# uci-rendering/psdr-cuda

Measured on AMD Instinct MI355X. Metric: Mpath-samples/s renderC+renderD, cbox 512x512 spp=64; grad rel-L2 vs ref, higher is better.
Workload: dtype f32; 1 GPU; cbox 512x512 spp=64/GPU PathTracer(max_depth=3): renderC + configure + renderD + enoki.forward w.r.t. diffuse albedo, through the psdr_cuda surface; triangles=12, global_spp=64, world_size=1, device=AMD Radeon Graphics, local_rank=0

## Files before the change

### psdr-cuda_amd/csrc/psdr_collocated.hip

```cpp
#ifndef PSDR_WIDE_TREE
#if PSDR_VARIANT_FLAGS == 6
#define PSDR_WIDE_TREE 1
#else
#define PSDR_WIDE_TREE 0
#endif
#endif
#ifndef PSDR_LEAF_PAIR
#if PSDR_VARIANT_FLAGS == 6
#define PSDR_LEAF_PAIR 1
#else
#define PSDR_LEAF_PAIR 0
#endif
#endif
#include "psdr_kernels.h"
#include "psdr_collocated.h"

#ifndef PSDR_VARIANT_FLAGS
#error "compile with -DPSDR_VARIANT_FLAGS=0|1|2|3|4|6|8|10"
#endif
#define PSDR_CAT2(a, b) a##b
#define PSDR_CAT(a, b) PSDR_CAT2(a, b)

namespace {

// ... 134 lines not shown
    const long long nceil = (n + kBlock - 1) / kBlock * kBlock;
    for (long long j = (long long) blockIdx.x * kBlock + threadIdx.x; j < nceil; j += (long long) gridDim.x * kBlock) {
        float w[4] = {0.f, 0.f, 0.f, 0.f};
        int edge = -1;
        if (j < n) edge = collocated_edge_reverse_values<FL>(cx.sc, st, cx.jump, (uint64_t) (i0 + (order ? (long long) order[j] : j)), inv_sppe, adj_img, nrays, w);
        const bool head = wave_run_sum<4>(edge, w);
        if (head && edge >= 0) {
#pragma unroll
            for (int i = 0; i < 4; ++i) sink.add_pedge(edge, i, w[i]);
        }
    }
    count_rays(counters, nrays);
}

template <class G, class R, int FL>
int colloc_run_camera(psdr_scene_s *h, const psdr_render_opts *o, const TV<R, FL> &tv, float *img, float *dimg, hipStream_t s) {
    const long long WH = (long long) h->desc.width * h->desc.height;
    const int nsp = o->spp_end - o->spp_begin;
    if (o->spp <= 0 || nsp <= 0) return 0;
    LaunchCtx cx;
    if (int rc = make_ctx(h, o, 0, cx)) return rc;
    const long long n = WH * nsp;
    h->slots[0] += (uint64_t) n;
    const int own = (h->opt.own_pixels != 0 && nsp <= 64 && 64 % nsp == 0) ? 1 : 0;
    hipLaunchKernelGGL(HIP_KERNEL_NAME(k_colloc_camera<G, R, FL>), dim3(launch_blocks(h, n, camera_blocks_per_cu(h, n))), dim3(kBlock), lds_bytes(cx, h), s, cx, tv, o->spp, o->spp_begin,
                       SlotDiv(nsp), n, 1.f / (float) o->spp, img, dimg, WH * 3, h->d_counters, own);
    HIP_TRY(hipGetLastError());
    return 0;
}

template <int FL>
int colloc_render_c(psdr_scene_s *h, const psdr_render_opts *o, float *out_img, hipStream_t s) {
    const TangentView<0, FL> tv0{};
    return colloc_run_camera<float, float, FL>(h, o, tv0, out_img, nullptr, s);
}

template <int K, int FL>
int colloc_render_fwd_k(psdr_scene_s *h, const psdr_render_opts *o, const psdr_tangents *tangents, float *img, float *dimg, hipStream_t s) {
    const long long WH = (long long) h->desc.width * h->desc.height;
    TangentView<K, FL> tv;
    for (int k = 0; k < K; ++k) tv.t[k] = tangents[k];
    HIP_TRY(hipMemsetAsync(img, 0, sizeof(float) * WH * 3, s));
    HIP_TRY(hipMemsetAsync(dimg, 0, sizeof(float) * WH * 3 * K, s));
    bool geo = false;
    for (int k = 0; k < K; ++k) geo = geo || tangents[k].d_tri_info || tangents[k].d_cam_to_world;
    if (geo) { if (int rc = colloc_run_camera<Dual<K>, Dual<K>, FL>(h, o, tv, img, dimg, s)) return rc; }
    else { if (int rc = colloc_run_camera<float, Dual<K>, FL>(h, o, tv, img, dimg, s)) return rc; }
// ... 95 lines not shown
```

### psdr-cuda_amd/csrc/psdr_hip.hip

```cpp
#define PSDR_WIDE_TREE 2
#include "psdr_host.h"
#include "psdr_bvh_build.h"

#include <cstdlib>
#include <cstring>
#include <rocprim/rocprim.hpp>

namespace {
__global__ __launch_bounds__(kBlock) void k_trace(LaunchCtx cx, int m, const float *__restrict__ ox, const float *__restrict__ oy,
                                                  const float *__restrict__ oz, const float *__restrict__ dx,
                                                  const float *__restrict__ dy, const float *__restrict__ dz,
                                                  const float *__restrict__ tmax, int32_t *__restrict__ out_shape,
                                                  int32_t *__restrict__ out_tri, float *__restrict__ out_u, float *__restrict__ out_v) {
    TraversalStack st; setup_lds(cx, st);
    const SceneView &sc = cx.sc;
    for (int i = blockIdx.x * kBlock + threadIdx.x; i < m; i += gridDim.x * kBlock) {
        const Hit h = closest_hit<false, -1>(sc, st, Vec3f{ox[i], oy[i], oz[i]}, Vec3f{dx[i], dy[i], dz[i]}, tmax[i]);
        out_tri[i] = h.tri;
        out_shape[i] = h.tri >= 0 ? (sc.d.tri_mesh[h.tri] & ~PSDR_TRI_FACE_NORMALS) : -1;
        out_u[i] = h.u; out_v[i] = h.v;
    }
}


// ... 527 lines not shown
    }
    return L;
}

int ensure_tree_kind(psdr_scene_s *h, hipStream_t s) {
    if (!h->have_bvh || h->num_nodes <= 0) return 0;
    if (forest_tables(h) && !small_tables_fit(h)) return psdr_bvh_build(h, s);
    const bool forest = h->n_blas > 0;
    if (use_wide_tree(h, forest) == h->wide) return 0;
    std::vector<BvhNode> host_nodes((size_t) h->num_nodes);
    HIP_TRY(hipMemcpyAsync(host_nodes.data(), h->d_nodes, host_nodes.size() * sizeof(BvhNode), hipMemcpyDeviceToHost, s));
    HIP_TRY(hipStreamSynchronize(s));
    std::vector<int32_t> roots;
    if (forest) for (int k = 0; k < h->n_blas; ++k) { int32_t r; std::memcpy(&r, &h->blas_lo[k].w, 4); roots.push_back(r); }
    else roots.push_back(h->root);
    return bvh4_build(h, host_nodes, roots, forest, s);
}

int begin_call(psdr_scene_s *h, hipStream_t s) {
    h->last_stream = s;
    if (int rc = ensure_tree_kind(h, s)) return rc;
    h->slots[0] = h->slots[1] = h->slots[2] = 0; h->last_path_depth = 0;
    HIP_TRY(hipMemsetAsync(h->d_counters, 0, sizeof(unsigned long long) * kRayCounters * kRayCounterStride, s));
    return 0;
}


int primary_edge_order(psdr_scene_s *h, const LaunchCtx &cx, long long i0, long long n, const uint32_t **order, hipStream_t s) {
    *order = nullptr;
    if (!h->sort_edges || n < 65536 || n > 0x7fffffffLL) return 0;
    size_t temp = 0;
    const unsigned long long tiles = (unsigned long long) ((cx.sc.d.width + 7) >> 3) * (unsigned long long) ((cx.sc.d.height + 7) >> 3);
    unsigned tile_bits = 0;
    while ((1ull << tile_bits) < tiles) ++tile_bits;
    if (tile_bits + 6 >= 32) return 0;
    const unsigned end_bit = tile_bits + 7;
    const uint32_t invalid_key = 1u << (tile_bits + 6);
    uint32_t *nul = nullptr;
    HIP_TRY(rocprim::radix_sort_pairs(nullptr, temp, nul, nul, nul, nul, (size_t) n, 0, end_bit, s));
    const size_t need = 4 * sizeof(uint32_t) * (size_t) n + temp + 256;
    if (int rc = scratch_reserve(&h->d_sort, &h->sort_bytes, need, s, "primary-edge sort scratch")) return rc;
    uint32_t *k_in = reinterpret_cast<uint32_t *>(h->d_sort), *k_out = k_in + n, *v_in = k_out + n, *v_out = v_in + n;
    void *tmp = reinterpret_cast<void *>((reinterpret_cast<uintptr_t>(v_out + n) + 255) & ~(uintptr_t) 255);
    hipLaunchKernelGGL(k_primary_edge_keys, dim3((unsigned) ((n + kBlock - 1) / kBlock)), dim3(kBlock), 0, s, cx.sc, cx.jump, i0, n, k_in, v_in, invalid_key);
    HIP_TRY(hipGetLastError());
    HIP_TRY(rocprim::radix_sort_pairs(tmp, temp, k_in, k_out, v_in, v_out, (size_t) n, 0, end_bit, s));
// ... 303 lines not shown
    else if (n == "emitter_pretest") h->opt.emitter_pretest = iv;
    else if (n == "occ_rows") { h->opt.occ_rows = iv; h->have_bvh = false; }
    else if (n == "aa_prims") { h->aa_enabled = iv != 0; h->have_bvh = false; }
    else if (n == "tiny_scene") h->tiny_enabled = iv != 0;
    else if (n == "two_level") h->two_level_enabled = iv != 0;
    else if (n == "wf_binned") h->wf_binned = iv != 0;
    else if (n == "wf_traced") h->traced_enabled = iv != 0;
    else if (n == "bvh_build") h->bvh_device_mode = iv;
    else if (n == "sort_edges") h->sort_edges = iv != 0;
    else if (n == "blocks_per_cu") h->opt.blocks_per_cu = iv;
    else if (n == "camera_blocks") h->opt.camera_blocks = iv;
    else if (n == "tiny_variants") h->opt.tiny_variants = iv;
    else if (n == "wide") h->opt.wide = iv;
    else if (n == "lds_budget") h->opt.lds_budget = iv;
    else if (n == "sink_rep") h->opt.sink_rep = std::max(1, std::min(16, iv));
    else if (n == "sink_private") h->opt.sink_private = iv;
    else if (n == "rev_split") h->opt.rev_split = iv;
    else if (n == "tangent_live") h->opt.tangent_live = iv;
    else if (n == "wf_geo") h->opt.wf_geo = iv;
    else if (n == "logd") h->opt.logd = iv;
    else if (n == "seed_cache") h->opt.seed_cache = iv;
    else if (n == "logd_park") h->opt.logd_park = iv;
    else if (n == "seed_cache_log2") h->opt.seed_cache_log2 = std::max(0, std::min(40, iv));
    else if (n == "keep_records") h->opt.keep_records = iv;
    else if (n == "rev_sorted") h->opt.rev_sorted = iv;
    else if (n == "sedge_split") h->opt.sedge_split = iv;
    else if (n == "pt_sedge") h->opt.pt_sedge = iv & 3;
    else if (n == "pt_sedge_walk") h->opt.pt_sedge_walk = iv;
    else if (n == "probe") h->opt.probe = iv;
    else if (n == "trace_wg2") h->opt.trace_wg2 = iv;
    else if (n == "chunk_log2") h->opt.chunk_log2 = std::max(0, std::min(30, iv));
    else if (n == "bvh_maxleaf") h->opt.bvh_maxleaf = std::max(1, std::min(8, iv));
    else if (n == "bvh_tcost") h->opt.bvh_tcost = (float) value;
    else return fail("psdr_scene_set_option: unknown option '" + n + "'");
    h->kept.valid = false;
    if (n == "tiny_scene" || n == "two_level" || n == "bvh_build" || n == "wide" || n == "bvh_maxleaf" || n == "bvh_tcost" || n == "tiny_variants") h->have_bvh = false;
    return 0;
}

int psdr_scene_destroy(psdr_scene_t h) {
    if (!h) return 0;
    if (h->d_nodes) (void) hipFree(h->d_nodes);
    if (h->d_btris) (void) hipFree(h->d_btris);
    if (h->d_counters) (void) hipFree(h->d_counters);
    if (h->d_refit_area) (void) hipFree(h->d_refit_area);
    if (h->d_sort) (void) hipFree(h->d_sort);
// ... 299 lines not shown
int psdr_trace(psdr_scene_t h, int32_t m, const float *ox, const float *oy, const float *oz, const float *dx, const float *dy,
               const float *dz, const float *tmax, int32_t *out_shape, int32_t *out_tri, float *out_u, float *out_v, void *stream) {
    if (!h || !h->have_tables) return fail("Scene not loaded yet!");
    if (!h->have_bvh) return fail("Input scene must be configured!");
    if (m <= 0) return 0;
    LaunchCtx cx{};
    cx.sc.d = h->desc; cx.sc.nodes = h->d_nodes; cx.sc.btris = h->d_btris; cx.sc.root = h->root;
    fill_top(h, cx.sc);
    plan_lds(h, cx);
    hipLaunchKernelGGL(k_trace, dim3(launch_blocks(h, m)), dim3(kBlock), lds_bytes(cx, h), (hipStream_t) stream, cx, m, ox, oy, oz, dx, dy, dz, tmax,
                       out_shape, out_tri, out_u, out_v);
    HIP_TRY(hipGetLastError());
    return 0;
}

int psdr_render_c(psdr_scene_t h, const psdr_render_opts *o, float *out_img, void *stream) {
    if (!h || !o || !out_img) return fail("psdr_render_c: null argument");
    if (!h->have_tables) return fail("Scene not loaded yet!");
    if (int rc = check_counts(h, o)) return rc;
    if (int rc = check_microfacet(h, o)) return rc;
    hipStream_t s = (hipStream_t) stream;
    if (int rc = begin_call(h, s)) return rc;
    if (o->integrator == PSDR_INTEGRATOR_PATH) h->last_path_depth = o->max_depth;
    const long long WH = (long long) h->desc.width * h->desc.height;
    HIP_TRY(hipMemsetAsync(out_img, 0, sizeof(float) * WH * 3, s));
    if (o->integrator == PSDR_INTEGRATOR_COLLOCATED) return collocated_of(h)->render_c(h, o, out_img, s);
    return variant_of(h)->render_c(h, o, out_img, s);
}

int psdr_render_d_fwd(psdr_scene_t h, const psdr_render_opts *o, int32_t K, const psdr_tangents *tangents, float *out_img,
                      float *out_dimg, void *stream) {
    if (!h || !o || !out_img || !out_dimg || !tangents) return fail("psdr_render_d_fwd: null argument");
    if (!h->have_tables) return fail("Scene not loaded yet!");
    if (int rc = check_counts(h, o)) return rc;
    if (int rc = check_microfacet(h, o)) return rc;
    if (int rc = check_path_sedges(o)) return rc;
    hipStream_t s = (hipStream_t) stream;
    if (int rc = begin_call(h, s)) return rc;
    if (K != 1 && K != 3) return fail("psdr_render_d_fwd: K must be 1 or 3");
    if (o->integrator == PSDR_INTEGRATOR_COLLOCATED) return collocated_of(h)->render_fwd(h, o, K, tangents, out_img, out_dimg, s);
    if (int rc = variant_of(h)->render_fwd(h, o, K, tangents, out_img, out_dimg, s)) return rc;
    return path_sedge_of(h)->fwd(h, o, K, tangents, out_dimg, s);
}

int psdr_render_d_rev(psdr_scene_t h, const psdr_render_opts *o, const float *adj_img, float *out_img, const psdr_grads *grads,
                      void *stream) {
    if (!h || !o || !adj_img || !grads) return fail("psdr_render_d_rev: null argument");
    if (!h->have_tables) return fail("Scene not loaded yet!");
    if (int rc = check_counts(h, o)) return rc;
// ... 158 lines not shown
```

### psdr-cuda_amd/csrc/psdr_host.h

```cpp
#pragma once
#include "psdr_device.h"
#include "psdr_reverse.h"

#include <algorithm>
#include <type_traits>
#include <cmath>
#include <cstdio>
#include <cstdlib>
#include <cstring>
#include <string>
#include <vector>

using namespace psdr;

struct LaunchCtx {
    SceneView sc;
    LiParams lp;
    RngJump jump;
    int32_t off_stack;
    int32_t off_pathrec;
    int32_t off_sink;
    int32_t off_park;
};

// ... 93 lines not shown
    int tiny_variants = 1;
    int wide = -1;
    int lds_budget = 0;
    int sink_rep = 4;
    int sink_private = 1;
    int rev_split = -1;
    int tangent_live = 1;
    int wf_geo = 1;
    int own_pixels = 1;
    int emitter_pretest = 1;
    int occ_rows = 1;
    int logd = 1;
    int keep_records = 1;
    int rev_sorted = 1;
    int pt_sedge = 3;
    int pt_sedge_walk = 1;
    int sedge_split = -1;
    int chunk_log2 = 0;
    int probe = 1;
    int trace_wg2 = -1;
    int seed_cache = 1;
    int seed_cache_log2 = 25;
    int logd_park = 1;
    int bvh_maxleaf = 4;
    float bvh_tcost = 2.0f;
};

struct psdr_scene_s {
    psdr_scene_options opt;
    psdr_scene_desc desc{};
    bool have_tables = false;
    bool has_rough = true;
    int num_cus = 256;
    int lds_limit = 64 * 1024;

    BvhNode *d_nodes = nullptr;
    float4 *d_btris = nullptr;
    size_t cap_nodes = 0, cap_btris = 0;
    int32_t root = 0;
    bool have_bvh = false;
    int bvh_depth = 0, num_nodes = 0, num_btris = 0;
    Bvh4Node *d_nodes4 = nullptr;
    int32_t *d_topo4 = nullptr;
    size_t cap_nodes4 = 0;
    int num_nodes4 = 0, stack_need4 = 0;
    bool wide = false;
// ... 33 lines not shown
    std::vector<int32_t> emitter_i;
    int32_t *d_hot_map = nullptr, *d_hot_tris = nullptr;
    uint32_t *d_occ = nullptr; size_t occ_cap = 0; bool have_occ = false; int occ_max_rows = 0;
    int hot_rows = 0;
    bool hot_identity = false;
    size_t hot_cap = 0;

    bool sort_edges = true;
    void *d_sort = nullptr;
    size_t sort_bytes = 0;

    void *d_pe_rep = nullptr;
    size_t pe_rep_bytes = 0;

    void *d_rev_deep = nullptr;
    size_t rev_deep_bytes = 0;

    void *d_se_list = nullptr;
    size_t se_list_bytes = 0;

    void *d_rev = nullptr;
    size_t rev_bytes = 0;
    void *d_logd_bad = nullptr; size_t logd_bad_bytes = 0;
    struct KeptRecords { bool valid = false; psdr_render_opts o{}; uint64_t gen = 0; long long n = 0; int kind = 0; } kept;
    uint64_t tables_gen = 0;

    void *d_seed = nullptr;
    size_t seed_cap = 0;
    long long seed_key[4] = {0, 0, 0, 0};
    bool seed_valid = false;
    hipStream_t seed_stream = nullptr;
    hipEvent_t seed_event = nullptr;
    long long seed_fills = 0, seed_launches = 0;
    long long logd_launches = 0, logd_lean_launches = 0, logd_lean_seeded = 0;
    int logd_lean_lds = 0, logd_lean_park = 0;
    void *d_ws = nullptr;
    size_t ws_bytes = 0;
    void *d_live = nullptr;
    size_t live_bytes = 0;
    void *d_probe = nullptr;
    size_t probe_bytes = 0;
    uint32_t emit_rows = 0;
    int forest_min_inline = 0;
    int32_t pg_reso[3] = {1, 1, 1};
    const float *pg_cmf = nullptr, *pg_pmf = nullptr;
    float pg_sum = 0.f;
// ... 79 lines not shown
```

### psdr-cuda_amd/csrc/psdr_kernels.h

```cpp
#pragma once
#include "psdr_host.h"

namespace {
using namespace psdr_host;

__device__ __forceinline__ float wave_shfl_down(float v, int off) { return __shfl_down(v, off, 64); }

template <int CTRL, int ROW_MASK> __device__ __forceinline__ float dpp_add(float v) {
    return v + __int_as_float(__builtin_amdgcn_update_dpp(0, __float_as_int(v), CTRL, ROW_MASK, 0xf, true));
}
__device__ __forceinline__ float wave_total(float v) {
    v = dpp_add<0x111, 0xf>(v); v = dpp_add<0x112, 0xf>(v); v = dpp_add<0x114, 0xf>(v); v = dpp_add<0x118, 0xf>(v);
    v = dpp_add<0x142, 0xa>(v); v = dpp_add<0x143, 0xc>(v);
    return __int_as_float(__builtin_amdgcn_readlane(__float_as_int(v), 63));
}
#ifndef PSDR_DPP_ALWAYS
#define PSDR_DPP_ALWAYS 0
#endif
template <int N, bool DPP = (N <= 6 || PSDR_DPP_ALWAYS)> __device__ __forceinline__ bool wave_segmented_sum(int key, float (&v)[N]) {
    const int lane = threadIdx.x & 63;
    if (DPP && __ballot(key != __builtin_amdgcn_readfirstlane(key)) == 0ull) {
#pragma unroll
        for (int i = 0; i < N; ++i) v[i] = wave_total(v[i]);
        return lane == 0;
// ... 161 lines not shown
                                                   unsigned long long *counters, int own, const ulonglong2 *__restrict__ seed) {
    static_assert((FL & kScenePre) == 0, "seeded launches have no probe rows");
    constexpr long long j0 = 0;
    const ProbeView pv{nullptr, nullptr};
    PSDR_CAMERA_KERNEL_BODY(PSDR_SEED_LOAD, (((void) slot), camera_sample<G, R, INTEG>(cx.sc, tv, st, cx.lp, seeded_rng(sd, cx.jump), pixel, nrays)))
}
#undef PSDR_CAMERA_KERNEL_BODY
#undef PSDR_SEED_LOAD
#undef PSDR_SEED_LOAD_NONE

template <int K>
__global__ __launch_bounds__(kBlock) void k_logd_check(const float *__restrict__ texels, TangentView<K, 0> tv, int n, unsigned long long *counters, int *bad) {
    const int i = blockIdx.x * kBlock + threadIdx.x;
    bool b = false;
    if (i < n) {
        bool moved = false;
#pragma unroll
        for (int k = 0; k < K; ++k) moved = moved || tv.t[k].d_texels[i] != 0.f;
        b = moved && !(fabsf(texels[i]) > 1e-20f);
    }
    if (__ballot(b) != 0ull && (threadIdx.x & 63) == 0) atomicOr(bad, 1);
}
__global__ void k_logd_gate(unsigned long long *counters, const int *bad) { if (threadIdx.x == 0 && blockIdx.x == 0) counters[kLogdGateWord] = *bad ? 0ull : 1ull; }
template <int K, int FL, bool NOTREE>
__global__ __launch_bounds__(kBlock, ((PSDR_LOGD_WAVES_K1 > 0 && K == 1 && NOTREE) ? PSDR_LOGD_WAVES_K1 : camera_waves<float, Dual<K>, PSDR_INTEGRATOR_PATH, FL, NOTREE>())) void k_camera_logd(LaunchCtx cx, TV<Dual<K>, FL> tv, int spp, int s_begin, SlotDiv nsp,
                                                   long long n, float inv_spp, float *__restrict__ img, float *__restrict__ dimg, long long plane, unsigned long long *counters, int own) {
    constexpr int NV = 3 * (1 + K);
    if (counters[kLogdGateWord] != 1ull) return;
    TraversalStack st; setup_lds(cx, st, tv);
    uint32_t nrays = 0;
    const long long nceil = (n + kBlock - 1) / kBlock * kBlock;
    for (long long j = (long long) blockIdx.x * kBlock + threadIdx.x; j < nceil; j += (long long) gridDim.x * kBlock) {
        const bool in = j < n;
        int pixel = 0x7fffffff, s_in = 0;
        if (in) slot_to_pixel(j, nsp, pixel, s_in);
        float v[NV];
#pragma unroll
        for (int i = 0; i < NV; ++i) v[i] = 0.f;
        if (in) {
            const uint64_t slot = (uint64_t) pixel * (uint64_t) spp + (uint64_t) (s_begin + s_in);
            const Vec3<Dual<K>> r = camera_sample_logd<K>(cx.sc, tv, st, cx.lp, cx.jump, pixel, slot, nrays);
            v[0] = r.x.v * inv_spp; v[1] = r.y.v * inv_spp; v[2] = r.z.v * inv_spp;
#pragma unroll
            for (int k = 0; k < K; ++k) { v[3 + 3 * k] = r.x.d[k] * inv_spp; v[4 + 3 * k] = r.y.d[k] * inv_spp; v[5 + 3 * k] = r.z.d[k] * inv_spp; }
        }
        const bool head = wave_segmented_sum<NV>(pixel, v);
// ... 1277 lines not shown
}
inline const ulonglong2 *seed_table(psdr_scene_s *h, const psdr_render_opts *o, long long WH, int nsp, long long n, hipStream_t s) {
    if (h->opt.seed_cache == 0 || n <= 0 || n > (1ll << std::max(0, std::min(40, h->opt.seed_cache_log2)))) return nullptr;
    const long long key[4] = {WH, (long long) o->spp, (long long) o->spp_begin, (long long) nsp};
    if (h->d_seed != nullptr && h->seed_valid && std::equal(key, key + 4, h->seed_key)) {
        if (s != h->seed_stream && h->seed_event != nullptr && hipStreamWaitEvent(s, h->seed_event, 0) != hipSuccess) { (void) hipGetLastError(); return nullptr; }
        return reinterpret_cast<const ulonglong2 *>(h->d_seed);
    }
    h->seed_valid = false;
    if ((size_t) n > h->seed_cap) {
        if (h->d_seed) { (void) hipFreeAsync(h->d_seed, s); h->d_seed = nullptr; h->seed_cap = 0; }
        void *nb = nullptr;
        if (hipMallocAsync(&nb, (size_t) n * sizeof(ulonglong2), s) != hipSuccess) { (void) hipGetLastError(); return nullptr; }
        h->d_seed = nb; h->seed_cap = (size_t) n;
    }
    if (h->seed_event == nullptr && hipEventCreateWithFlags(&h->seed_event, hipEventDisableTiming) != hipSuccess) { (void) hipGetLastError(); h->seed_event = nullptr; return nullptr; }
    hipLaunchKernelGGL(k_seed_fill, dim3((unsigned) ((n + kBlock - 1) / kBlock)), dim3(kBlock), 0, s, reinterpret_cast<ulonglong2 *>(h->d_seed), n, o->spp, o->spp_begin, SlotDiv(nsp));
    if (hipGetLastError() != hipSuccess || hipEventRecord(h->seed_event, s) != hipSuccess) { (void) hipGetLastError(); return nullptr; }
    std::copy(key, key + 4, h->seed_key);
    h->seed_valid = true; h->seed_stream = s; h->seed_fills++;
    return reinterpret_cast<const ulonglong2 *>(h->d_seed);
}
template <class G, class R, int FL> constexpr bool seeded_render_c() { return (FL & kSceneTiny) != 0 && (FL & kScenePre) == 0 && std::is_same<G, float>::value && std::is_same<R, float>::value; }
template <class G, class R, int FL>
int run_camera(psdr_scene_s *h, const psdr_render_opts *o, const TV<R, FL> &tv, float *img, float *dimg, hipStream_t s) {
    const long long WH = (long long) h->desc.width * h->desc.height;
    const int nsp = o->spp_end - o->spp_begin;
    if (o->spp <= 0 || nsp <= 0) return 0;
    LaunchCtx cx;
    if (int rc = make_ctx(h, o, 0, cx)) return rc;
    const long long n = WH * nsp;
    h->slots[0] += (uint64_t) n;
    const int own = (h->opt.own_pixels != 0 && nsp <= 64 && 64 % nsp == 0) ? 1 : 0;
    if constexpr ((FL & kSceneForest) != 0) {
        if (o->integrator == PSDR_INTEGRATOR_DIRECT && probe_direct(h, o, n)) {
            const TangentView<0, FL> tv0{};
            TV<R, FL | kScenePre> tvp;
            for (int k = 0; k < (ad_traits<R>::K > 0 ? ad_traits<R>::K : 1); ++k) tvp.t[k] = tv.t[k];
            tvp.live = tv.live;
            LaunchCtx cxp = cx;
            plan_lds(h, cxp, 1 << 30);
            cxp.sc.n_lnodes = cxp.sc.n_lbtris = cxp.sc.n_ltri = 0;
            const long long chunk = std::min<long long>(n, launch_chunk(h, 25));
            for (long long c0 = 0; c0 < n; c0 += chunk) {
                const long long nc = std::min(chunk, n - c0);
                ProbeBuffers pb;
                const int probe_per_cu = big_launch_per_cu(h, nc);
                if (int rc = probe_buffers(h, nc, 3, pb, s, probe_per_cu)) return rc;
                const TraceQueue tq{pb.req, pb.count, pb.sub_cap};
                const int blocks = (launch_blocks(h, nc, probe_per_cu) + kWfSub - 1) / kWfSub * kWfSub;
                hipLaunchKernelGGL(k_direct_probe<FL>, dim3(blocks), dim3(kBlock), lds_bytes(cx, h), s, cx, tv0, o->spp, o->spp_begin, SlotDiv(nsp), c0, nc, tq, pb.hit, pb.mask,
                                   make_rng_jump(o->rng_offset[0] + 2));
                HIP_TRY(hipGetLastError());
                if (int rc = launch_wf_trace(h, pb.req, pb.count, pb.sub_cap, pb.hit, s)) return rc;
                hipLaunchKernelGGL(HIP_KERNEL_NAME(k_camera<G, R, PSDR_INTEGRATOR_DIRECT, FL | kScenePre, false>), dim3(launch_blocks(h, nc, camera_blocks_per_cu(h, nc))), dim3(kBlock), cxp.off_stack, s,
                                   cxp, tvp, o->spp, o->spp_begin, SlotDiv(nsp), nc, 1.f / (float) o->spp, img, dimg, WH * 3, h->d_counters, c0, ProbeView{pb.hit, pb.mask}, own);
                HIP_TRY(hipGetLastError());
            }
            return 0;
        }
    }
    bool gated = false;
    if constexpr (logd_instance<G, R, PSDR_INTEGRATOR_PATH, FL>()) {
        constexpr int K = ad_traits<R>::K;
        bool texels_only = o->integrator == PSDR_INTEGRATOR_PATH && h->opt.logd != 0 && h->desc.num_texels > 0 && h->desc.texels != nullptr;
        for (int k = 0; k < K && texels_only; ++k) {
            const psdr_tangents &t = tv.t[k];
            texels_only = t.d_texels != nullptr && !t.d_tri_info && !t.d_emitter_rad && !t.d_cam_to_world && !t.d_sec_edge && !t.d_prim_edge && !t.d_env_f;
        }
        if (texels_only) {
            if (int rc = scratch_reserve(&h->d_logd_bad, &h->logd_bad_bytes, sizeof(int), s, "log-derivative gate")) return rc;
            int *bad = reinterpret_cast<int *>(h->d_logd_bad);
            HIP_TRY(hipMemsetAsync(bad, 0, sizeof(int), s));
            TangentView<K, 0> tvk;
            for (int k = 0; k < K; ++k) tvk.t[k] = tv.t[k];
            hipLaunchKernelGGL(k_logd_check<K>, dim3((unsigned) ((h->desc.num_texels + kBlock - 1) / kBlock)), dim3(kBlock), 0, s, h->desc.texels, tvk, h->desc.num_texels, h->d_counters, bad);
            hipLaunchKernelGGL(k_logd_gate, dim3(1), dim3(64), 0, s, h->d_counters, bad);
            bool lean = false;
            if constexpr (K == 1 && FL == kSceneTiny) { if (int rc = logd_lean_launch_8(h, o, cx, tv, img, dimg, s, &lean)) return rc; }
            if (!lean)
                hipLaunchKernelGGL(HIP_KERNEL_NAME(k_camera_logd<K, FL, ((FL & kSceneTiny) != 0)>), dim3(launch_blocks(h, n, camera_blocks_per_cu(h, n))), dim3(kBlock), lds_bytes(cx, h), s, cx, tv,
                                   o->spp, o->spp_begin, SlotDiv(nsp), n, 1.f / (float) o->spp, img, dimg, WH * 3, h->d_counters, own);
            HIP_TRY(hipGetLastError());
            h->logd_launches++;
            gated = true;
        }
    }
#define PSDR_LAUNCH_CAMERA_T(INTEG, NOTREE)                                                                                        \
    hipLaunchKernelGGL(HIP_KERNEL_NAME(k_camera<G, R, INTEG, FL, NOTREE>), dim3(launch_blocks(h, n, camera_blocks_per_cu(h, n))), dim3(kBlock), lds_bytes(cx, h), s, cx, tv, o->spp, \
                       o->spp_begin, nsp, n, 1.f / (float) o->spp, img, dimg, WH * 3, h->d_counters, 0ll, ProbeView{nullptr, nullptr}, own)
#define PSDR_LAUNCH_CAMERA(INTEG) PSDR_LAUNCH_CAMERA_T(INTEG, ((FL & kSceneTiny) != 0))
    if constexpr (seeded_render_c<G, R, FL>()) {
        if (o->integrator == PSDR_INTEGRATOR_PATH) {
            if (const ulonglong2 *seed = seed_table(h, o, WH, nsp, n, s)) {
                hipLaunchKernelGGL(HIP_KERNEL_NAME(k_camera_seeded<G, R, PSDR_INTEGRATOR_PATH, FL, true>), dim3(launch_blocks(h, n, camera_blocks_per_cu(h, n))), dim3(kBlock), lds_bytes(cx, h), s, cx, tv,
                                   o->spp, o->spp_begin, SlotDiv(nsp), n, 1.f / (float) o->spp, img, dimg, WH * 3, h->d_counters, own, seed);
                HIP_TRY(hipGetLastError());
                h->seed_launches++;
                return 0;
            }
        }
    }
    switch (o->integrator) {
        case PSDR_INTEGRATOR_DIRECT: PSDR_LAUNCH_CAMERA(PSDR_INTEGRATOR_DIRECT); break;
        case PSDR_INTEGRATOR_PATH: PSDR_LAUNCH_CAMERA(PSDR_INTEGRATOR_PATH); break;
        case PSDR_INTEGRATOR_FIELD: PSDR_LAUNCH_CAMERA(PSDR_INTEGRATOR_FIELD); break;
        default: return fail("Unknown integrator");
    }
#undef PSDR_LAUNCH_CAMERA
#undef PSDR_LAUNCH_CAMERA_T
    HIP_TRY(hipGetLastError());
    if (gated) HIP_TRY(hipMemsetAsync(h->d_counters + kLogdGateWord, 0, sizeof(unsigned long long), s));
    return 0;
}


constexpr int kWfMaxDepth = 256;
struct WfRecArgs { float *disk; long long stride, c0, nc; };
template <class M, int FL>
int run_camera_wavefront(psdr_scene_s *h, const psdr_render_opts *o, const TV<M, FL> &tv, float *img, float *dimg, hipStream_t s, const WfRecArgs *rec = nullptr) {
    constexpr int K = ad_traits<M>::K;
    const long long WH = (long long) h->desc.width * h->desc.height;
    const int nsp = o->spp_end - o->spp_begin;
    if (o->spp <= 0 || nsp <= 0) return 0;
    const long long n_all = WH * nsp;
    const long long n = rec ? rec->nc : n_all;
    bool traced = false;
    if constexpr ((FL & kSceneForest) != 0) traced = traced_wavefront(h);
    const bool binned = !traced && (FL & kSceneForest) != 0 && h->n_blas > 0 && h->wf_binned;
    const int depth = o->max_depth;
    const size_t words = 8 + 6 * (1 + K) + (traced ? 8 : 0);
    const long long cap = rec ? n : std::min(n, fit_chunk(binned ? launch_chunk(h, 24) : launch_chunk(h, traced ? 26 : 25), 2 * words * 4 * 5 / 4 + (traced ? 80 : 0), 64u << 20, h->ws_bytes));
    const auto wf_per_cu = [&](long long slots) { return traced ? big_launch_per_cu(h, slots) : 16; };
    const long long max_blocks = ((long long) launch_blocks(h, cap, wf_per_cu(cap)) + kWfSub - 1) / kWfSub * kWfSub;
    const long long binned_sub_cap = (((cap + kBlock - 1) / kBlock + kWfSub) / kWfGroups + 2) * kBlock;
// ... 210 lines not shown

struct TangentRows { const float *p[3]; };
__global__ __launch_bounds__(kBlock) void k_tangent_live(TangentRows tr, int K, int T, uint32_t *__restrict__ live) {
    const int tri = blockIdx.x * kBlock + threadIdx.x;
    bool any = false;
    if (tri < T) {
        for (int k = 0; k < K; ++k) {
            const float *p = tr.p[k];
            if (p == nullptr) continue;
            const float4 *q = reinterpret_cast<const float4 *>(p + (size_t) tri * PSDR_TRI_STRIDE);
#pragma unroll
            for (int i = 0; i < PSDR_TRI_STRIDE / 4; ++i) { const float4 v = q[i]; any = any || v.x != 0.f || v.y != 0.f || v.z != 0.f || v.w != 0.f; }
        }
    }
    const unsigned long long m = __ballot(any);
    if ((threadIdx.x & 63) == 0 && tri < T) { live[tri >> 5] = (uint32_t) m; live[(tri >> 5) + 1] = (uint32_t) (m >> 32); }
}

template <int K, int FL>
int render_fwd(psdr_scene_s *h, const psdr_render_opts *o, const psdr_tangents *tangents, float *img, float *dimg, hipStream_t s) {
    const long long WH = (long long) h->desc.width * h->desc.height;
    TangentView<K, FL> tv;
    for (int k = 0; k < K; ++k) tv.t[k] = tangents[k];
    HIP_TRY(hipMemsetAsync(img, 0, sizeof(float) * WH * 3, s));
    HIP_TRY(hipMemsetAsync(dimg, 0, sizeof(float) * WH * 3 * K, s));
    bool geo = false;
    for (int k = 0; k < K; ++k) geo = geo || tangents[k].d_tri_info || tangents[k].d_cam_to_world;
    if (geo && PSDR_TANGENT_LIVE && h->opt.tangent_live != 0) {
        static_assert(K <= 3, "TangentRows holds three sets");
        const int T = h->desc.num_tris;
        const size_t need = ((size_t) (T + 63) / 64 * 2 + 2) * sizeof(uint32_t);
        if (int rc = scratch_reserve(&h->d_live, &h->live_bytes, need, s, "tangent liveness mask")) return rc;
        TangentRows tr{};
        for (int k = 0; k < K; ++k) tr.p[k] = tangents[k].d_tri_info;
        hipLaunchKernelGGL(k_tangent_live, dim3((unsigned) ((T + kBlock - 1) / kBlock)), dim3(kBlock), 0, s, tr, K, T, reinterpret_cast<uint32_t *>(h->d_live));
        HIP_TRY(hipGetLastError());
        tv.live = reinterpret_cast<const uint32_t *>(h->d_live);
    }
    bool geo_wavefront = false;
    if constexpr ((FL & kSceneForest) != 0) geo_wavefront = geo && h->opt.wf_geo != 0 && traced_wavefront(h) && use_wavefront(h, o);
    if (geo_wavefront) {
        if constexpr ((FL & kSceneForest) != 0) { if (int rc = run_camera_wavefront_geo<K, FL>(h, o, tv, img, dimg, s)) return rc; }
    } else if (geo) { if (int rc = run_camera<Dual<K>, Dual<K>, FL>(h, o, tv, img, dimg, s)) return rc; }
    else if (use_wavefront(h, o)) { if (int rc = run_camera_wavefront<Dual<K>, FL>(h, o, tv, img, dimg, s)) return rc; }
    else { if (int rc = run_camera<float, Dual<K>, FL>(h, o, tv, img, dimg, s)) return rc; }
    if (o->sppe > 0 && o->sppe_end > o->sppe_begin && h->desc.num_prim_edges > 0) {
        LaunchCtx cx;
        if (int rc = make_ctx(h, o, 1, cx)) return rc;
        const long long i0 = WH * o->sppe_begin, n = WH * (o->sppe_end - o->sppe_begin);
        h->slots[1] += (uint64_t) n;
        const uint32_t *order = nullptr;
        if (int rc = primary_edge_order(h, cx, i0, n, &order, s)) return rc;
#define PSDR_LAUNCH_PE(INTEG)                                                                                                        \
        hipLaunchKernelGGL(HIP_KERNEL_NAME(k_primary_edge<K, FL, INTEG>), dim3(launch_blocks(h, n)), dim3(kBlock), lds_bytes(cx, h), s, cx, tv, i0, n,   \
                           1.f / (float) o->sppe, dimg, WH * 3, h->d_counters, order)
        switch (o->integrator) {
            case PSDR_INTEGRATOR_DIRECT: PSDR_LAUNCH_PE(PSDR_INTEGRATOR_DIRECT); break;
            case PSDR_INTEGRATOR_PATH: PSDR_LAUNCH_PE(PSDR_INTEGRATOR_PATH); break;
            default: PSDR_LAUNCH_PE(PSDR_INTEGRATOR_FIELD); break;
        }
#undef PSDR_LAUNCH_PE
        HIP_TRY(hipGetLastError());
    }
    if (o->sppse > 0 && o->sppse_end > o->sppse_begin && h->desc.num_sec_edges > 0 && o->integrator == PSDR_INTEGRATOR_DIRECT) {
        LaunchCtx cx;
        if (int rc = make_ctx(h, o, 2, cx)) return rc;
        const long long i0 = WH * o->sppse_begin, n = WH * (o->sppse_end - o->sppse_begin);
        h->slots[2] += (uint64_t) n;
// ... 261 lines not shown
                       out_mass, h->d_counters);
    HIP_TRY(hipGetLastError());
    return 0;
}

template <int FL>
int render_rev(psdr_scene_s *h, const psdr_render_opts *o, const float *adj_img, float *out_img, const psdr_grads *grads, hipStream_t s) {
    return render_rev_impl<FL>(h, o, adj_img, out_img, grads, s, false);
}

template <int FL>
int render_c_launch(psdr_scene_s *h, const psdr_render_opts *o, float *out_img, hipStream_t s) {
    const TangentView<0, FL> tv0{};
    if constexpr ((FL & kSceneForest) != 0) {
        const long long n = (long long) h->desc.width * h->desc.height * (o->spp_end - o->spp_begin);
        const int depth_k = std::min(o->max_depth, kMaxRevDepthDeep);
        if ((o->flags & PSDR_FLAG_KEEP_RECORDS) != 0 && h->opt.keep_records != 0 && o->spp > 0 && n > 0 && n <= launch_chunk(h, 26) && rev_value_sweep_is_wavefront<FL>(h, o, n) &&
            n <= fit_chunk(std::max(n, 1ll << 18), (size_t) rev_record_words(h, depth_k, true) * 4 + 240, 128u << 20, h->rev_bytes + h->ws_bytes)) {
            const int depth = depth_k;
            const size_t need = (size_t) n * rev_record_words(h, depth, true) * sizeof(float);
            h->kept.valid = false;
            if (int rc = scratch_reserve(&h->d_rev, &h->rev_bytes, need, s, "per-path records of the split reverse launch")) return rc;
            const WfRecArgs ra{reinterpret_cast<float *>(h->d_rev), n, 0, n};
            if (int rc = run_camera_wavefront<float, FL>(h, o, tv0, out_img, nullptr, s, &ra)) return rc;
            h->slots[0] += (uint64_t) n;
            h->kept.valid = true; h->kept.o = *o; h->kept.gen = h->tables_gen; h->kept.n = n; h->kept.kind = 1;
            return 0;
        }
    }
    if ((o->flags & PSDR_FLAG_KEEP_RECORDS) != 0 && h->opt.keep_records != 0 && !use_wavefront(h, o)) {
        const psdr_grads none{};
        const int rc = render_rev_impl<FL>(h, o, nullptr, out_img, &none, s, true);
        if (rc != 1) return rc;
    }
    if (use_wavefront(h, o)) return run_camera_wavefront<float, FL>(h, o, tv0, out_img, nullptr, s);
    return run_camera<float, float, FL>(h, o, tv0, out_img, nullptr, s);
}

template <int FL>
int render_fwd_launch(psdr_scene_s *h, const psdr_render_opts *o, int K, const psdr_tangents *tangents, float *img, float *dimg, hipStream_t s) {
    switch (K) {
        case 1: return render_fwd<1, FL>(h, o, tangents, img, dimg, s);
        case 3: return render_fwd<3, FL>(h, o, tangents, img, dimg, s);
        default: return fail("psdr_render_d_fwd: K must be 1 or 3");
    }
}

}
```

### psdr-cuda_amd/csrc/psdr_logd_lean.hip

```cpp
#define PSDR_WIDE_TREE 0
#define PSDR_LEAF_PAIR 0
#include "psdr_kernels.h"
#include "psdr_logd_lean.h"

namespace {

constexpr int kLeanFlags = kSceneTiny;

template <int K, int FL, bool SEEDED>
__global__ __launch_bounds__(kBlock, PSDR_LOGD_WAVES_K1) void k_camera_logd_lean(LaunchCtx cx, TV<Dual<K>, FL> tv, int spp, int s_begin, SlotDiv nsp, long long n, float inv_spp,
                                                                                  float *__restrict__ img, float *__restrict__ dimg, long long plane, unsigned long long *counters, int own,
                                                                                  const ulonglong2 *__restrict__ seed) {
    constexpr int NV = 3 * (1 + K);
    if (counters[kLogdGateWord] != 1ull) return;
    TraversalStack st; setup_lds(cx, st, tv);
    Park pk{nullptr};
#if defined(__HIP_DEVICE_COMPILE__)
    pk.base = reinterpret_cast<float *>(psdr_dyn_lds + cx.off_park) + threadIdx.x;
#endif
    uint32_t nrays = 0;
    const long long nceil = (n + kBlock - 1) / kBlock * kBlock;
    for (long long jb = (long long) blockIdx.x * kBlock; jb < nceil; jb += (long long) gridDim.x * kBlock) {
        const long long j = jb + threadIdx.x;
        const bool in = j < n;
// ... 35 lines not shown
                    if (v[5 + 3 * k] != 0.f) atomicAdd(q + 2, v[5 + 3 * k]);
                }
            }
        }
    }
    count_rays(counters, nrays);
}

}

namespace psdr_host {
int logd_lean_launch_8(psdr_scene_s *h, const psdr_render_opts *o, const LaunchCtx &cx0, const psdr::TangentView<1, psdr::kSceneTiny> &tv, float *img, float *dimg, hipStream_t s, bool *ran) {
    *ran = false;
    if (h->opt.logd_park == 0) return 0;
    constexpr int kCuLds = 160 * 1024, park = ParkLayout<1>::cols * kBlock * 4;
    const int lds = (lds_bytes(cx0, h) + 15) / 16 * 16;
    const int limit = h->opt.lds_budget > 0 ? std::min(h->opt.lds_budget, kCuLds / PSDR_LOGD_WAVES_K1) : kCuLds / PSDR_LOGD_WAVES_K1;
    if (lds + park > limit) return 0;
    LaunchCtx cx = cx0;
    cx.off_park = lds;
    const long long WH = (long long) h->desc.width * h->desc.height;
    const int nsp = o->spp_end - o->spp_begin;
    const long long n = WH * nsp;
    const int own = (h->opt.own_pixels != 0 && nsp <= 64 && 64 % nsp == 0) ? 1 : 0;
    const dim3 grid(launch_blocks(h, n, camera_blocks_per_cu(h, n)));
    const ulonglong2 *seed = seed_table(h, o, WH, nsp, n, s);
    if (seed != nullptr)
        hipLaunchKernelGGL(HIP_KERNEL_NAME(k_camera_logd_lean<1, kLeanFlags, true>), grid, dim3(kBlock), lds + park, s, cx, tv, o->spp, o->spp_begin, SlotDiv(nsp), n, 1.f / (float) o->spp, img, dimg,
                           WH * 3, h->d_counters, own, seed);
    else
        hipLaunchKernelGGL(HIP_KERNEL_NAME(k_camera_logd_lean<1, kLeanFlags, false>), grid, dim3(kBlock), lds + park, s, cx, tv, o->spp, o->spp_begin, SlotDiv(nsp), n, 1.f / (float) o->spp, img, dimg,
                           WH * 3, h->d_counters, own, seed);
    h->logd_lean_launches++;
    if (seed != nullptr) { h->logd_lean_seeded++; h->seed_launches++; }
    h->logd_lean_lds = lds; h->logd_lean_park = park;
    *ran = true;
    return 0;
}
}
```

Baseline: 20640 Mpath-samples/s.

## Skip redundant image memsets and fuse log-derivative gate into one small kernel

The image and derivative-image memsets are dropped when the camera kernel owns every pixel and writes it directly, and are kept only on the wavefront, probe and non-owning paths. For small texel counts, the scratch reserve, memset, check kernel and gate kernel of the log-derivative gate become a single one-block kernel. The gate-word reset after the camera launch is deferred to the next PATH call that does not use the gate. This removes several small launches and memsets per render, at the cost of extra state and a risk of stale image data or a stale gate if the ownership assumptions fail.

```diff
diff --git a/psdr-cuda_amd/csrc/psdr_collocated.hip b/psdr-cuda_amd/csrc/psdr_collocated.hip
--- a/psdr-cuda_amd/csrc/psdr_collocated.hip
+++ b/psdr-cuda_amd/csrc/psdr_collocated.hip
@@ -180,7 +180,7 @@
     if (int rc = make_ctx(h, o, 0, cx)) return rc;
     const long long n = WH * nsp;
     h->slots[0] += (uint64_t) n;
-    const int own = (h->opt.own_pixels != 0 && nsp <= 64 && 64 % nsp == 0) ? 1 : 0;
+    const int own = camera_stores_image(h, o) ? 1 : 0;
     hipLaunchKernelGGL(HIP_KERNEL_NAME(k_colloc_camera<G, R, FL>), dim3(launch_blocks(h, n, camera_blocks_per_cu(h, n))), dim3(kBlock), lds_bytes(cx, h), s, cx, tv, o->spp, o->spp_begin,
                        SlotDiv(nsp), n, 1.f / (float) o->spp, img, dimg, WH * 3, h->d_counters, own);
     HIP_TRY(hipGetLastError());
diff --git a/psdr-cuda_amd/csrc/psdr_hip.hip b/psdr-cuda_amd/csrc/psdr_hip.hip
--- a/psdr-cuda_amd/csrc/psdr_hip.hip
+++ b/psdr-cuda_amd/csrc/psdr_hip.hip
@@ -573,6 +573,7 @@
     if (int rc = ensure_tree_kind(h, s)) return rc;
     h->slots[0] = h->slots[1] = h->slots[2] = 0; h->last_path_depth = 0;
     HIP_TRY(hipMemsetAsync(h->d_counters, 0, sizeof(unsigned long long) * kRayCounters * kRayCounterStride, s));
+    h->logd_gate_open = false;
     return 0;
 }
 
@@ -922,6 +923,9 @@
     else if (n == "seed_cache") h->opt.seed_cache = iv;
     else if (n == "logd_park") h->opt.logd_park = iv;
     else if (n == "seed_cache_log2") h->opt.seed_cache_log2 = std::max(0, std::min(40, iv));
+    else if (n == "zero_skip") h->opt.zero_skip = iv;
+    else if (n == "logd_gate_fused") h->opt.logd_gate_fused = iv;
+    else if (n == "logd_gate_bound") h->opt.logd_gate_bound = std::max(0, iv);
     else if (n == "keep_records") h->opt.keep_records = iv;
     else if (n == "rev_sorted") h->opt.rev_sorted = iv;
     else if (n == "sedge_split") h->opt.sedge_split = iv;
@@ -1267,9 +1271,11 @@
     hipStream_t s = (hipStream_t) stream;
     if (int rc = begin_call(h, s)) return rc;
     if (o->integrator == PSDR_INTEGRATOR_PATH) h->last_path_depth = o->max_depth;
-    const long long WH = (long long) h->desc.width * h->desc.height;
-    HIP_TRY(hipMemsetAsync(out_img, 0, sizeof(float) * WH * 3, s));
-    if (o->integrator == PSDR_INTEGRATOR_COLLOCATED) return collocated_of(h)->render_c(h, o, out_img, s);
+    if (o->integrator == PSDR_INTEGRATOR_COLLOCATED) {
+        const long long WH = (long long) h->desc.width * h->desc.height;
+        HIP_TRY(hipMemsetAsync(out_img, 0, sizeof(float) * WH * 3, s));
+        return collocated_of(h)->render_c(h, o, out_img, s);
+    }
     return variant_of(h)->render_c(h, o, out_img, s);
 }
 
diff --git a/psdr-cuda_amd/csrc/psdr_host.h b/psdr-cuda_amd/csrc/psdr_host.h
--- a/psdr-cuda_amd/csrc/psdr_host.h
+++ b/psdr-cuda_amd/csrc/psdr_host.h
@@ -139,6 +139,9 @@
     int seed_cache = 1;
     int seed_cache_log2 = 25;
     int logd_park = 1;
+    int zero_skip = 1;
+    int logd_gate_fused = 1;
+    int logd_gate_bound = 1 << 13;
     int bvh_maxleaf = 4;
     float bvh_tcost = 2.0f;
 };
@@ -218,6 +221,7 @@
     void *d_rev = nullptr;
     size_t rev_bytes = 0;
     void *d_logd_bad = nullptr; size_t logd_bad_bytes = 0;
+    bool logd_gate_open = false;
     struct KeptRecords { bool valid = false; psdr_render_opts o{}; uint64_t gen = 0; long long n = 0; int kind = 0; } kept;
     uint64_t tables_gen = 0;
 
diff --git a/psdr-cuda_amd/csrc/psdr_kernels.h b/psdr-cuda_amd/csrc/psdr_kernels.h
--- a/psdr-cuda_amd/csrc/psdr_kernels.h
+++ b/psdr-cuda_amd/csrc/psdr_kernels.h
@@ -207,6 +207,18 @@
     if (__ballot(b) != 0ull && (threadIdx.x & 63) == 0) atomicOr(bad, 1);
 }
 __global__ void k_logd_gate(unsigned long long *counters, const int *bad) { if (threadIdx.x == 0 && blockIdx.x == 0) counters[kLogdGateWord] = *bad ? 0ull : 1ull; }
+template <int K>
+__global__ __launch_bounds__(kBlock) void k_logd_gate_small(const float *__restrict__ texels, TangentView<K, 0> tv, int n, unsigned long long *counters) {
+    bool b = false;
+    for (int i = threadIdx.x; i < n; i += kBlock) {
+        bool moved = false;
+#pragma unroll
+        for (int k = 0; k < K; ++k) moved = moved || tv.t[k].d_texels[i] != 0.f;
+        b = b || (moved && !(fabsf(texels[i]) > 1e-20f));
+    }
+    const int bad = __syncthreads_or(b ? 1 : 0);
+    if (threadIdx.x == 0) counters[kLogdGateWord] = bad ? 0ull : 1ull;
+}
 template <int K, int FL, bool NOTREE>
 __global__ __launch_bounds__(kBlock, ((PSDR_LOGD_WAVES_K1 > 0 && K == 1 && NOTREE) ? PSDR_LOGD_WAVES_K1 : camera_waves<float, Dual<K>, PSDR_INTEGRATOR_PATH, FL, NOTREE>())) void k_camera_logd(LaunchCtx cx, TV<Dual<K>, FL> tv, int spp, int s_begin, SlotDiv nsp,
                                                    long long n, float inv_spp, float *__restrict__ img, float *__restrict__ dimg, long long plane, unsigned long long *counters, int own) {
@@ -1530,18 +1542,32 @@
     return reinterpret_cast<const ulonglong2 *>(h->d_seed);
 }
 template <class G, class R, int FL> constexpr bool seeded_render_c() { return (FL & kSceneTiny) != 0 && (FL & kScenePre) == 0 && std::is_same<G, float>::value && std::is_same<R, float>::value; }
+inline bool camera_stores_image(const psdr_scene_s *h, const psdr_render_opts *o) {
+    const int nsp = o->spp_end - o->spp_begin;
+    return h->opt.own_pixels != 0 && o->spp > 0 && nsp > 0 && nsp <= 64 && 64 % nsp == 0;
+}
+inline int zero_images(const psdr_scene_s *h, float *img, float *dimg, int K, hipStream_t s) {
+    const size_t bytes = sizeof(float) * 3 * (size_t) h->desc.width * (size_t) h->desc.height;
+    HIP_TRY(hipMemsetAsync(img, 0, bytes, s));
+    if (K > 0) HIP_TRY(hipMemsetAsync(dimg, 0, bytes * K, s));
+    return 0;
+}
 template <class G, class R, int FL>
 int run_camera(psdr_scene_s *h, const psdr_render_opts *o, const TV<R, FL> &tv, float *img, float *dimg, hipStream_t s) {
     const long long WH = (long long) h->desc.width * h->desc.height;
     const int nsp = o->spp_end - o->spp_begin;
+    const long long n = WH * nsp;
+    bool probe = false;
+    if constexpr ((FL & kSceneForest) != 0) probe = o->spp > 0 && nsp > 0 && o->integrator == PSDR_INTEGRATOR_DIRECT && probe_direct(h, o, n);
+    const bool stores = camera_stores_image(h, o);
+    if (probe || !stores || h->opt.zero_skip == 0) { if (int rc = zero_images(h, img, dimg, ad_traits<R>::K, s)) return rc; }
     if (o->spp <= 0 || nsp <= 0) return 0;
     LaunchCtx cx;
     if (int rc = make_ctx(h, o, 0, cx)) return rc;
-    const long long n = WH * nsp;
     h->slots[0] += (uint64_t) n;
-    const int own = (h->opt.own_pixels != 0 && nsp <= 64 && 64 % nsp == 0) ? 1 : 0;
+    const int own = stores ? 1 : 0;
     if constexpr ((FL & kSceneForest) != 0) {
-        if (o->integrator == PSDR_INTEGRATOR_DIRECT && probe_direct(h, o, n)) {
+        if (probe) {
             const TangentView<0, FL> tv0{};
             TV<R, FL | kScenePre> tvp;
             for (int k = 0; k < (ad_traits<R>::K > 0 ? ad_traits<R>::K : 1); ++k) tvp.t[k] = tv.t[k];
@@ -1550,6 +1576,7 @@
             plan_lds(h, cxp, 1 << 30);
             cxp.sc.n_lnodes = cxp.sc.n_lbtris = cxp.sc.n_ltri = 0;
             const long long chunk = std::min<long long>(n, launch_chunk(h, 25));
+            const int own_chunk = (own && (chunk >= n || chunk % 64 == 0)) ? 1 : 0;
             for (long long c0 = 0; c0 < n; c0 += chunk) {
                 const long long nc = std::min(chunk, n - c0);
                 ProbeBuffers pb;
@@ -1562,7 +1589,7 @@
                 HIP_TRY(hipGetLastError());
                 if (int rc = launch_wf_trace(h, pb.req, pb.count, pb.sub_cap, pb.hit, s)) return rc;
                 hipLaunchKernelGGL(HIP_KERNEL_NAME(k_camera<G, R, PSDR_INTEGRATOR_DIRECT, FL | kScenePre, false>), dim3(launch_blocks(h, nc, camera_blocks_per_cu(h, nc))), dim3(kBlock), cxp.off_stack, s,
-                                   cxp, tvp, o->spp, o->spp_begin, SlotDiv(nsp), nc, 1.f / (float) o->spp, img, dimg, WH * 3, h->d_counters, c0, ProbeView{pb.hit, pb.mask}, own);
+                                   cxp, tvp, o->spp, o->spp_begin, SlotDiv(nsp), nc, 1.f / (float) o->spp, img, dimg, WH * 3, h->d_counters, c0, ProbeView{pb.hit, pb.mask}, own_chunk);
                 HIP_TRY(hipGetLastError());
             }
             return 0;
@@ -1577,13 +1604,17 @@
             texels_only = t.d_texels != nullptr && !t.d_tri_info && !t.d_emitter_rad && !t.d_cam_to_world && !t.d_sec_edge && !t.d_prim_edge && !t.d_env_f;
         }
         if (texels_only) {
-            if (int rc = scratch_reserve(&h->d_logd_bad, &h->logd_bad_bytes, sizeof(int), s, "log-derivative gate")) return rc;
-            int *bad = reinterpret_cast<int *>(h->d_logd_bad);
-            HIP_TRY(hipMemsetAsync(bad, 0, sizeof(int), s));
             TangentView<K, 0> tvk;
             for (int k = 0; k < K; ++k) tvk.t[k] = tv.t[k];
-            hipLaunchKernelGGL(k_logd_check<K>, dim3((unsigned) ((h->desc.num_texels + kBlock - 1) / kBlock)), dim3(kBlock), 0, s, h->desc.texels, tvk, h->desc.num_texels, h->d_counters, bad);
-            hipLaunchKernelGGL(k_logd_gate, dim3(1), dim3(64), 0, s, h->d_counters, bad);
+            if (h->opt.logd_gate_fused != 0 && h->desc.num_texels <= h->opt.logd_gate_bound) {
+                hipLaunchKernelGGL(k_logd_gate_small<K>, dim3(1), dim3(kBlock), 0, s, h->desc.texels, tvk, h->desc.num_texels, h->d_counters);
+            } else {
+                if (int rc = scratch_reserve(&h->d_logd_bad, &h->logd_bad_bytes, sizeof(int), s, "log-derivative gate")) return rc;
+                int *bad = reinterpret_cast<int *>(h->d_logd_bad);
+                HIP_TRY(hipMemsetAsync(bad, 0, sizeof(int), s));
+                hipLaunchKernelGGL(k_logd_check<K>, dim3((unsigned) ((h->desc.num_texels + kBlock - 1) / kBlock)), dim3(kBlock), 0, s, h->desc.texels, tvk, h->desc.num_texels, h->d_counters, bad);
+                hipLaunchKernelGGL(k_logd_gate, dim3(1), dim3(64), 0, s, h->d_counters, bad);
+            }
             bool lean = false;
             if constexpr (K == 1 && FL == kSceneTiny) { if (int rc = logd_lean_launch_8(h, o, cx, tv, img, dimg, s, &lean)) return rc; }
             if (!lean)
@@ -1592,6 +1623,9 @@
             HIP_TRY(hipGetLastError());
             h->logd_launches++;
             gated = true;
+        } else if (o->integrator == PSDR_INTEGRATOR_PATH && h->logd_gate_open) {
+            HIP_TRY(hipMemsetAsync(h->d_counters + kLogdGateWord, 0, sizeof(unsigned long long), s));
+            h->logd_gate_open = false;
         }
     }
 #define PSDR_LAUNCH_CAMERA_T(INTEG, NOTREE)                                                                                        \
@@ -1618,7 +1652,10 @@
 #undef PSDR_LAUNCH_CAMERA
 #undef PSDR_LAUNCH_CAMERA_T
     HIP_TRY(hipGetLastError());
-    if (gated) HIP_TRY(hipMemsetAsync(h->d_counters + kLogdGateWord, 0, sizeof(unsigned long long), s));
+    if (gated) {
+        if (h->opt.logd_gate_fused != 0) h->logd_gate_open = true;
+        else HIP_TRY(hipMemsetAsync(h->d_counters + kLogdGateWord, 0, sizeof(unsigned long long), s));
+    }
     return 0;
 }
 
@@ -1875,8 +1912,6 @@
     const long long WH = (long long) h->desc.width * h->desc.height;
     TangentView<K, FL> tv;
     for (int k = 0; k < K; ++k) tv.t[k] = tangents[k];
-    HIP_TRY(hipMemsetAsync(img, 0, sizeof(float) * WH * 3, s));
-    HIP_TRY(hipMemsetAsync(dimg, 0, sizeof(float) * WH * 3 * K, s));
     bool geo = false;
     for (int k = 0; k < K; ++k) geo = geo || tangents[k].d_tri_info || tangents[k].d_cam_to_world;
     if (geo && PSDR_TANGENT_LIVE && h->opt.tangent_live != 0) {
@@ -1893,10 +1928,13 @@
     bool geo_wavefront = false;
     if constexpr ((FL & kSceneForest) != 0) geo_wavefront = geo && h->opt.wf_geo != 0 && traced_wavefront(h) && use_wavefront(h, o);
     if (geo_wavefront) {
+        if (int rc = zero_images(h, img, dimg, K, s)) return rc;
         if constexpr ((FL & kSceneForest) != 0) { if (int rc = run_camera_wavefront_geo<K, FL>(h, o, tv, img, dimg, s)) return rc; }
     } else if (geo) { if (int rc = run_camera<Dual<K>, Dual<K>, FL>(h, o, tv, img, dimg, s)) return rc; }
-    else if (use_wavefront(h, o)) { if (int rc = run_camera_wavefront<Dual<K>, FL>(h, o, tv, img, dimg, s)) return rc; }
-    else { if (int rc = run_camera<float, Dual<K>, FL>(h, o, tv, img, dimg, s)) return rc; }
+    else if (use_wavefront(h, o)) {
+        if (int rc = zero_images(h, img, dimg, K, s)) return rc;
+        if (int rc = run_camera_wavefront<Dual<K>, FL>(h, o, tv, img, dimg, s)) return rc;
+    } else { if (int rc = run_camera<float, Dual<K>, FL>(h, o, tv, img, dimg, s)) return rc; }
     if (o->sppe > 0 && o->sppe_end > o->sppe_begin && h->desc.num_prim_edges > 0) {
         LaunchCtx cx;
         if (int rc = make_ctx(h, o, 1, cx)) return rc;
@@ -2204,6 +2242,7 @@
             h->kept.valid = false;
             if (int rc = scratch_reserve(&h->d_rev, &h->rev_bytes, need, s, "per-path records of the split reverse launch")) return rc;
             const WfRecArgs ra{reinterpret_cast<float *>(h->d_rev), n, 0, n};
+            if (int rc = zero_images(h, out_img, nullptr, 0, s)) return rc;
             if (int rc = run_camera_wavefront<float, FL>(h, o, tv0, out_img, nullptr, s, &ra)) return rc;
             h->slots[0] += (uint64_t) n;
             h->kept.valid = true; h->kept.o = *o; h->kept.gen = h->tables_gen; h->kept.n = n; h->kept.kind = 1;
@@ -2215,7 +2254,10 @@
         const int rc = render_rev_impl<FL>(h, o, nullptr, out_img, &none, s, true);
         if (rc != 1) return rc;
     }
-    if (use_wavefront(h, o)) return run_camera_wavefront<float, FL>(h, o, tv0, out_img, nullptr, s);
+    if (use_wavefront(h, o)) {
+        if (int rc = zero_images(h, out_img, nullptr, 0, s)) return rc;
+        return run_camera_wavefront<float, FL>(h, o, tv0, out_img, nullptr, s);
+    }
     return run_camera<float, float, FL>(h, o, tv0, out_img, nullptr, s);
 }
 
diff --git a/psdr-cuda_amd/csrc/psdr_logd_lean.hip b/psdr-cuda_amd/csrc/psdr_logd_lean.hip
--- a/psdr-cuda_amd/csrc/psdr_logd_lean.hip
+++ b/psdr-cuda_amd/csrc/psdr_logd_lean.hip
@@ -81,7 +81,7 @@
     const long long WH = (long long) h->desc.width * h->desc.height;
     const int nsp = o->spp_end - o->spp_begin;
     const long long n = WH * nsp;
-    const int own = (h->opt.own_pixels != 0 && nsp <= 64 && 64 % nsp == 0) ? 1 : 0;
+    const int own = camera_stores_image(h, o) ? 1 : 0;
     const dim3 grid(launch_blocks(h, n, camera_blocks_per_cu(h, n)));
     const ulonglong2 *seed = seed_table(h, o, WH, nsp, n, s);
     if (seed != nullptr)
```

New measurement: 20730 Mpath-samples/s (median of 6 runs). Within noise of the previous version (+0.4%).
